# skyepurchase/MeatModeler

Measured on AMD Instinct MI355X. Metric: descriptor-match pairs/sec + BA residuals/sec, 500×1080p frames, 1/2/4/8 GPU, higher is better.
Workload: dtype u8/int32 (match), f64 (BA); 1 GPU; 500 frames 1920x1080, 4000 ORB kpts/frame, BF Hamming 2-NN + ratio, track linking, 2-view DLT, full BA (TRF, Schur, f64 MFMA Cholesky); frames=500, height=1080, width=1920, nfeatures=4000, parallelism=pairs/points x1

## Files before the change

meatmodeler_amd/csrc/schur.hip:

```cpp
#include "ba_eval.h"
#include "chol_init.h"

namespace {

constexpr int SR_WIN = 256;

__global__ __launch_bounds__(256) void point_inverse_kernel(int P, const double *__restrict__ Cd,
                                                            double *__restrict__ Cinv) {
    int p = blockIdx.x * 256 + threadIdx.x;
    if (p >= P) return;
    const double *c = Cd + (size_t)p * 6;
    const double a = c[0], b = c[1], d = c[2], e = c[3], f = c[4], g = c[5];
    const double m00 = e * g - f * f, m01 = d * f - b * g, m02 = b * f - d * e;
    const double det = a * m00 + b * m01 + d * m02;
    const double id = 1.0 / det;
    double *o = Cinv + (size_t)p * 6;
    o[0] = m00 * id;
    o[1] = m01 * id;
    o[2] = m02 * id;
    o[3] = (a * g - d * d) * id;
    o[4] = (b * d - a * f) * id;
    o[5] = (a * e - b * b) * id;
}

// ... 35 lines not shown
        }
        if (blockIdx.y == 0) {
            const double g0 = gp[(size_t)p * 3], g1 = gp[(size_t)p * 3 + 1], g2 = gp[(size_t)p * 3 + 2];
#pragma unroll
            for (int a = 0; a < 6; ++a) vg[a] += Y[a][0] * g0 + Y[a][1] * g1 + Y[a][2] * g2;
        }
        for (int e2i = pb.pt_ptr[p]; e2i < pb.pt_ptr[p + 1]; ++e2i) {
            const int o2 = pb.pt_obs[e2i];
            const int f2 = pb.fi[o2];
            if (f2 < w0 || f2 >= w0 + wn) continue;
            Proj p2;
            ba_eval<true, true>(cams + (size_t)f2 * 6, Xp, Ks, pb.obs[2 * (size_t)o2], pb.obs[2 * (size_t)o2 + 1], p2);
            double *dst = &acc[0][(f2 - w0) * 6];
#pragma unroll
            for (int b = 0; b < 6; ++b) {
                const double e0 = p2.Jc[0][b] * p2.Jp[0][0] + p2.Jc[1][b] * p2.Jp[1][0];
                const double e1 = p2.Jc[0][b] * p2.Jp[0][1] + p2.Jc[1][b] * p2.Jp[1][1];
                const double e2 = p2.Jc[0][b] * p2.Jp[0][2] + p2.Jc[1][b] * p2.Jp[1][2];
#pragma unroll
                for (int a = 0; a < 6; ++a)
                    atomicAdd(dst + a * (SR_WIN * 6) + b, Y[a][0] * e0 + Y[a][1] * e1 + Y[a][2] * e2);
            }
        }
    }
    __syncthreads();
    for (int e = threadIdx.x; e < 6 * wn * 6; e += 256) {
        const int a = e / (wn * 6), c = e % (wn * 6);
        const int col = w0 * 6 + c;
        double val = -acc[a][c];
        if (col / 6 == i) val += Bd[(size_t)i * 36 + a * 6 + (col % 6)];
        S[((size_t)i * 6 + a) * n + col] = val;
    }
    if (blockIdx.y == 0) {
#pragma unroll
        for (int a = 0; a < 6; ++a) {
            const double s = block_sum<256>(vg[a], sm);
            if (threadIdx.x == 0) v[(size_t)i * 6 + a] = gc[(size_t)i * 6 + a] - s;
        }
    }
}

#ifndef MM_SP_WAVES
#define MM_SP_WAVES 1
#endif
constexpr int SP_WAVES = MM_SP_WAVES;
constexpr int MAX_SLABS = 64;
struct SlabSync {
    int32_t *ready;
    int32_t *done;
    int32_t seg_count[MAX_SLABS];
    int cams_per_slab;
};
constexpr int CAMTAB = 11;
__device__ __forceinline__ void write_chunk_desc(const mm_ba_problem &pb, int32_t *__restrict__ desc, int64_t first, int64_t stride) {
    for (int64_t k = first; k < pb.n_chunks; k += stride) {
        const int sidx = pb.chunk_seg[k], seg = pb.seg_ids[sidx];
        const int ci = seg / (pb.cam_span + 1), cdd = seg % (pb.cam_span + 1);
        const int c_first = pb.seg_chunk_ptr[sidx];
        int32_t *o = desc + 8 * k;
        o[0] = ci;
        o[1] = ci - cdd;
        o[2] = pb.chunk_begin[k];
        o[3] = pb.chunk_end[k];
        o[4] = sidx;
        o[5] = c_first;
        o[6] = pb.seg_chunk_ptr[sidx + 1] - c_first;
        o[7] = 0;
    }
}
__global__ __launch_bounds__(64) void cam_table_kernel(int F, const double *__restrict__ cams, double *__restrict__ tab,
                                                       int32_t *__restrict__ seg_done, int64_t n_seg, const double *__restrict__ K_lean,
                                                       mm_ba_problem pb, int32_t *__restrict__ desc) {
    const int f = blockIdx.x * 64 + threadIdx.x;
    for (int64_t k = f; k < n_seg; k += (int64_t)gridDim.x * 64) seg_done[k] = 0;
    if (desc) write_chunk_desc(pb, desc, f, (int64_t)gridDim.x * 64);
    if (f >= F) return;
    const double *c = cams + (size_t)f * 6;
    if (K_lean) {
        cam_table2_row(c, K_lean, tab + (size_t)f * CAMTAB2);
        return;
    }
    const CamCoef k = cam_coef_of(c);
    double *t = tab + (size_t)f * CAMTAB;
    for (int q = 0; q < 6; ++q) t[q] = c[q];
    t[6] = k.c;
    t[7] = k.a;
    t[8] = k.b;
    t[9] = k.a1;
    t[10] = k.b1;
}

__device__ __forceinline__ CamVals cam_vals_from_table(const double *__restrict__ t) {
    CamVals v;
    v.rx = uniform_f64(t[0]);
    v.ry = uniform_f64(t[1]);
    v.rz = uniform_f64(t[2]);
    v.tx = uniform_f64(t[3]);
    v.ty = uniform_f64(t[4]);
    v.tz = uniform_f64(t[5]);
    v.k.c = uniform_f64(t[6]);
    v.k.a = uniform_f64(t[7]);
    v.k.b = uniform_f64(t[8]);
    v.k.a1 = uniform_f64(t[9]);
    v.k.b1 = uniform_f64(t[10]);
    return v;
}

constexpr int RED_LD = 65;
__device__ __forceinline__ void wave_lds_barrier() {
    __builtin_amdgcn_fence(__ATOMIC_RELEASE, "wavefront");
    __builtin_amdgcn_wave_barrier();
    __builtin_amdgcn_fence(__ATOMIC_ACQUIRE, "wavefront");
}
__device__ __forceinline__ void wave_reduce_42(const double (&acc)[42], double *slab , int lane, double &out0,
                                               double &out1) {
#pragma unroll
    for (int h = 0; h < 2; ++h) {
#pragma unroll
        for (int q = 0; q < 21; ++q) slab[q * RED_LD + lane] = acc[21 * h + q];
        wave_lds_barrier();
        double s = 0.0;
        if (lane < 21) {
            const double *row = slab + lane * RED_LD;
            double s0 = 0.0, s1 = 0.0, s2 = 0.0, s3 = 0.0;
#pragma unroll
            for (int j = 0; j < 64; j += 4) {
                s0 += row[j];
                s1 += row[j + 1];
// ... 118 lines not shown
        if (writer && lane < 21) {
            tot0 = 0.0;
            tot1 = 0.0;
            for (int cc = 0; cc < n_ch; ++cc) {
                tot0 += __hip_atomic_load(partial + (size_t)(c_first + cc) * 42 + lane, __ATOMIC_RELAXED, __HIP_MEMORY_SCOPE_AGENT);
                tot1 += __hip_atomic_load(partial + (size_t)(c_first + cc) * 42 + 21 + lane, __ATOMIC_RELAXED, __HIP_MEMORY_SCOPE_AGENT);
            }
        }
    }
    if (!writer) return;
    if (lane < 21) {
#pragma unroll
        for (int h = 0; h < 2; ++h) {
            const int q = 21 * h + lane;
            const double sum = h == 0 ? tot0 : tot1;
            if (q < 36) {
                double val = -sum;
                if (d == 0) val += Bd[(size_t)i * 36 + q];
                __hip_atomic_store(S + ((size_t)i * 6 + q / 6) * n + (size_t)f2 * 6 + q % 6, val, __ATOMIC_RELAXED, __HIP_MEMORY_SCOPE_AGENT);
                if (d != 0)
                    __hip_atomic_store(S + ((size_t)f2 * 6 + q % 6) * n + (size_t)i * 6 + q / 6, val, __ATOMIC_RELAXED, __HIP_MEMORY_SCOPE_AGENT);
            } else if (d == 0) {
                __hip_atomic_store(v + (size_t)i * 6 + (q - 36), gc[(size_t)i * 6 + (q - 36)] - sum, __ATOMIC_RELAXED, __HIP_MEMORY_SCOPE_AGENT);
            }
        }
    }
    if (slabs.ready) {
        asm volatile("s_waitcnt vmcnt(0)" ::: "memory");
        __builtin_amdgcn_wave_barrier();
        if (lane == 0) {
            const int sl = i / slabs.cams_per_slab;
            if (atomicAdd(slabs.done + sl, 1) == slabs.seg_count[sl] - 1)
                __hip_atomic_store(slabs.ready + sl, 1, __ATOMIC_RELEASE, __HIP_MEMORY_SCOPE_AGENT);
        }
    }
}


struct CamPQ {
    double P[9], q[3];
};
__device__ __forceinline__ double fast_rcp(double x) {
    double y = __builtin_amdgcn_rcp(x);
    double e = fma(-x, y, 1.0);
    y = fma(y, e, y);
    e = fma(-x, y, 1.0);
    return fma(y, e, y);
}

struct LeanJ {
    double Jc[2][6];
    double Jp[2][3];
};
__device__ __forceinline__ void lean_eval(const CamPQ &c, const double *__restrict__ Ks, const double *__restrict__ Jr,
                                          double X0, double X1, double X2, LeanJ &o) {
    const double u0 = fma(c.P[0], X0, fma(c.P[1], X1, fma(c.P[2], X2, c.q[0])));
    const double u1 = fma(c.P[3], X0, fma(c.P[4], X1, fma(c.P[5], X2, c.q[1])));
    const double u2 = fma(c.P[6], X0, fma(c.P[7], X1, fma(c.P[8], X2, c.q[2])));
    const double iz = fast_rcp(u2);
    const double p[2] = {u0 * iz, u1 * iz};
#pragma unroll
    for (int m = 0; m < 2; ++m) {
#pragma unroll
        for (int k = 0; k < 3; ++k) {
            o.Jp[m][k] = fma(-p[m], c.P[6 + k], c.P[3 * m + k]) * iz;
            o.Jc[m][3 + k] = fma(-p[m], Ks[6 + k], Ks[3 * m + k]) * iz;
        }
        const double g0 = X1 * o.Jp[m][2] - X2 * o.Jp[m][1];
        const double g1 = X2 * o.Jp[m][0] - X0 * o.Jp[m][2];
        const double g2 = X0 * o.Jp[m][1] - X1 * o.Jp[m][0];
#pragma unroll
        for (int k = 0; k < 3; ++k) o.Jc[m][k] = fma(g0, Jr[k], fma(g1, Jr[3 + k], g2 * Jr[6 + k]));
    }
}

constexpr int SLAB2 = 32;
struct ChunkDesc {
    int32_t i, f2, e_begin, e_end, sidx, c_first, n_ch, pad;
};
template <bool FORCE>
__device__ __forceinline__ CamPQ cam_pq_scalar(const double *__restrict__ t) {
    CamPQ v;
#pragma unroll
    for (int k = 0; k < 9; ++k) v.P[k] = FORCE ? uniform_f64(t[k]) : t[k];
#pragma unroll
    for (int k = 0; k < 3; ++k) v.q[k] = FORCE ? uniform_f64(t[9 + k]) : t[9 + k];
    return v;
}
template <bool FORCE_UNIFORM>
__device__ __forceinline__ void schur_pairs_body(const mm_ba_problem pb, const double *__restrict__ camtab,
                                                                    const ChunkDesc *__restrict__ desc,
                                                                    const double *__restrict__ pts,
                                                                    const double *__restrict__ Cinv,
                                                                    const double *__restrict__ gp,
                                                                    double *partial, const double *__restrict__ Bd,
                                                                    const double *__restrict__ gc, double *S, double *v,
                                                                    int32_t *seg_done, SlabSync slabs, unsigned wg_begin,
                                                                    unsigned wg_total, const unsigned bx) {
    __shared__ double Ks[9];
    __shared__ double red[SP_WAVES][21 * RED_LD];
    __shared__ double jrs[SP_WAVES][SLAB2];
    if (threadIdx.x < 9) Ks[threadIdx.x] = pb.K[threadIdx.x];
    const int lane = threadIdx.x & 63;
    const int wv = __builtin_amdgcn_readfirstlane((int)(threadIdx.x >> 6));
    const unsigned gpos = bx + wg_begin;
    const unsigned wg = (gpos & 1) ? wg_total - 1 - (gpos >> 1) : (gpos >> 1);
    const int64_t c = (int64_t)wg * SP_WAVES + wv;
    const bool live = c < pb.n_chunks;
    ChunkDesc cd = {};
    if (live) cd = desc[c];
    if (FORCE_UNIFORM) {
        cd.i = __builtin_amdgcn_readfirstlane(cd.i);
        cd.f2 = __builtin_amdgcn_readfirstlane(cd.f2);
        cd.e_begin = __builtin_amdgcn_readfirstlane(cd.e_begin);
        cd.e_end = __builtin_amdgcn_readfirstlane(cd.e_end);
        cd.sidx = __builtin_amdgcn_readfirstlane(cd.sidx);
        cd.c_first = __builtin_amdgcn_readfirstlane(cd.c_first);
        cd.n_ch = __builtin_amdgcn_readfirstlane(cd.n_ch);
    }
    const int i = cd.i, f2 = cd.f2, d = cd.i - cd.f2, sidx = cd.sidx;
    const int e_begin = cd.e_begin, e_end = cd.e_end;
    auto point_of = [&](int e) { return pb.pair_p ? pb.pair_p[e] : pb.pi[pb.pair_o[e]]; };
    auto self_of = [&](int e) { return d == 0 && pb.pair_o[e] == pb.pair_o2[e]; };
    int e = e_begin + lane;
    int p_next = -1;
    bool self_next = false;
    if (live) {
        if (e < e_end) {
            p_next = point_of(e);
            self_next = self_of(e);
        }
        if (lane < 9) jrs[wv][lane] = camtab[(size_t)i * CAMTAB2 + 12 + lane];
        else if (lane >= 16 && lane < 25) jrs[wv][lane] = camtab[(size_t)f2 * CAMTAB2 + 12 + lane - 16];
    }
    __syncthreads();
    if (!live) return;
    const CamPQ cp_i = cam_pq_scalar<FORCE_UNIFORM>(camtab + (size_t)i * CAMTAB2), cp_2 = cam_pq_scalar<FORCE_UNIFORM>(camtab + (size_t)f2 * CAMTAB2);
    const double *Jr_i = jrs[wv], *Jr_2 = jrs[wv] + 16;
    double acc[42];
#pragma unroll
    for (int q = 0; q < 42; ++q) acc[q] = 0.0;
    auto load_xc = [&](int p, double (&x)[12]) {
        if (p >= 0) {
            const double *Xp = pts + (size_t)p * 3, *ci = Cinv + (size_t)p * 6;
            x[0] = Xp[0];
            x[1] = Xp[1];
            x[2] = Xp[2];
#pragma unroll
            for (int q = 0; q < 6; ++q) x[3 + q] = ci[q];
            if (d == 0) {
                x[9] = gp[(size_t)p * 3];
                x[10] = gp[(size_t)p * 3 + 1];
                x[11] = gp[(size_t)p * 3 + 2];
            }
        }
    };
    auto pair_body = [&](int p, bool self, const double (&x)[12]) {
        const double X0 = x[0], X1 = x[1], X2 = x[2];
        const double q00 = x[3], q01 = x[4], q02 = x[5], q11 = x[6], q12 = x[7], q22 = x[8];
        LeanJ a;
        lean_eval(cp_i, Ks, Jr_i, X0, X1, X2, a);
        double Z[2][3];
#pragma unroll
        for (int m = 0; m < 2; ++m) {
            Z[m][0] = a.Jp[m][0] * q00 + a.Jp[m][1] * q01 + a.Jp[m][2] * q02;
            Z[m][1] = a.Jp[m][0] * q01 + a.Jp[m][1] * q11 + a.Jp[m][2] * q12;
            Z[m][2] = a.Jp[m][0] * q02 + a.Jp[m][1] * q12 + a.Jp[m][2] * q22;
        }
        double M[2][2], T[2][6];
        if (d == 0) {
            if (self) {
                const double g0 = x[9], g1 = x[10], g2 = x[11];
                const double z0 = Z[0][0] * g0 + Z[0][1] * g1 + Z[0][2] * g2, z1 = Z[1][0] * g0 + Z[1][1] * g1 + Z[1][2] * g2;
#pragma unroll
                for (int q = 0; q < 6; ++q) acc[36 + q] += a.Jc[0][q] * z0 + a.Jc[1][q] * z1;
            }
#pragma unroll
            for (int m = 0; m < 2; ++m)
#pragma unroll
                for (int n_ = 0; n_ < 2; ++n_) M[m][n_] = Z[m][0] * a.Jp[n_][0] + Z[m][1] * a.Jp[n_][1] + Z[m][2] * a.Jp[n_][2];
#pragma unroll
            for (int b = 0; b < 6; ++b) {
                T[0][b] = M[0][0] * a.Jc[0][b] + M[0][1] * a.Jc[1][b];
                T[1][b] = M[1][0] * a.Jc[0][b] + M[1][1] * a.Jc[1][b];
            }
        } else {
            LeanJ b2;
            lean_eval(cp_2, Ks, Jr_2, X0, X1, X2, b2);
#pragma unroll
            for (int m = 0; m < 2; ++m)
#pragma unroll
                for (int n_ = 0; n_ < 2; ++n_) M[m][n_] = Z[m][0] * b2.Jp[n_][0] + Z[m][1] * b2.Jp[n_][1] + Z[m][2] * b2.Jp[n_][2];
#pragma unroll
            for (int b = 0; b < 6; ++b) {
                T[0][b] = M[0][0] * b2.Jc[0][b] + M[0][1] * b2.Jc[1][b];
                T[1][b] = M[1][0] * b2.Jc[0][b] + M[1][1] * b2.Jc[1][b];
            }
        }
#pragma unroll
        for (int q = 0; q < 6; ++q)
#pragma unroll
            for (int b = 0; b < 6; ++b) acc[q * 6 + b] += a.Jc[0][q] * T[0][b] + a.Jc[1][q] * T[1][b];
    };
    double xc[12];
    load_xc(p_next, xc);
    int p_cur = p_next;
    bool self_cur = self_next;
    {
        const int en = e + 64;
        p_next = en < e_end ? point_of(en) : -1;
        self_next = en < e_end && self_of(en);
    }
#pragma clang loop unroll(disable)
    for (; e - lane < e_end; e += 64) {
        double xn[12];
        load_xc(p_next, xn);
        const int p_nn_e = e + 128;
        const int p_nn = p_nn_e < e_end ? point_of(p_nn_e) : -1;
        const bool self_nn = p_nn_e < e_end && self_of(p_nn_e);
        if (p_cur >= 0) pair_body(p_cur, self_cur, xc);
#pragma unroll
        for (int q = 0; q < 12; ++q) xc[q] = xn[q];
        p_cur = p_next;
        self_cur = self_next;
        p_next = p_nn;
        self_next = self_nn;
    }
    double tot0, tot1;
    wave_reduce_42(acc, red[wv], lane, tot0, tot1);
    const int c_first = cd.c_first, n_ch = cd.n_ch;
    const size_t n = (size_t)pb.F * 6;
    bool writer = true;
    if (n_ch > 1) {
        if (lane < 21) {
            __hip_atomic_store(partial + (size_t)c * 42 + lane, tot0, __ATOMIC_RELAXED, __HIP_MEMORY_SCOPE_AGENT);
            __hip_atomic_store(partial + (size_t)c * 42 + 21 + lane, tot1, __ATOMIC_RELAXED, __HIP_MEMORY_SCOPE_AGENT);
        }
        asm volatile("s_waitcnt vmcnt(0)" ::: "memory");
        __builtin_amdgcn_wave_barrier();
        int last = 0;
        if (lane == 0) last = atomicAdd(seg_done + sidx, 1) == n_ch - 1;
        writer = __shfl(last, 0, 64) != 0;
        if (writer && lane < 21) {
            tot0 = 0.0;
            tot1 = 0.0;
            for (int cc = 0; cc < n_ch; ++cc) {
                tot0 += __hip_atomic_load(partial + (size_t)(c_first + cc) * 42 + lane, __ATOMIC_RELAXED, __HIP_MEMORY_SCOPE_AGENT);
                tot1 += __hip_atomic_load(partial + (size_t)(c_first + cc) * 42 + 21 + lane, __ATOMIC_RELAXED, __HIP_MEMORY_SCOPE_AGENT);
            }
        }
    }
    if (!writer) return;
    const bool through = slabs.ready != nullptr;
    if (lane < 21) {
#pragma unroll
        for (int h = 0; h < 2; ++h) {
            const int q = 21 * h + lane;
            const double sum = h == 0 ? tot0 : tot1;
            if (q < 36) {
                double val = -sum;
                if (d == 0) val += Bd[(size_t)i * 36 + q];
                double *dst = S + ((size_t)i * 6 + q / 6) * n + (size_t)f2 * 6 + q % 6;
                double *mir = S + ((size_t)f2 * 6 + q % 6) * n + (size_t)i * 6 + q / 6;
                if (through) {
                    __hip_atomic_store(dst, val, __ATOMIC_RELAXED, __HIP_MEMORY_SCOPE_AGENT);
                    if (d != 0) __hip_atomic_store(mir, val, __ATOMIC_RELAXED, __HIP_MEMORY_SCOPE_AGENT);
                } else {
                    *dst = val;
                    if (d != 0) *mir = val;
                }
            } else if (d == 0) {
                double *dst = v + (size_t)i * 6 + (q - 36);
                const double val = gc[(size_t)i * 6 + (q - 36)] - sum;
                if (through) __hip_atomic_store(dst, val, __ATOMIC_RELAXED, __HIP_MEMORY_SCOPE_AGENT);
                else *dst = val;
            }
        }
    }
    if (slabs.ready) {
        asm volatile("s_waitcnt vmcnt(0)" ::: "memory");
        __builtin_amdgcn_wave_barrier();
        if (lane == 0) {
            const int sl = i / slabs.cams_per_slab;
            if (atomicAdd(slabs.done + sl, 1) == slabs.seg_count[sl] - 1)
// ... 6 lines not shown
                                                                    const ChunkDesc *__restrict__ desc,
                                                                    const double *__restrict__ pts,
                                                                    const double *__restrict__ Cinv,
                                                                    const double *__restrict__ gp,
                                                                    double *partial, const double *__restrict__ Bd,
                                                                    const double *__restrict__ gc, double *S, double *v,
                                                                    int32_t *seg_done, SlabSync slabs, unsigned wg_begin,
                                                                    unsigned wg_total) {
    schur_pairs_body<false>(pb, camtab, desc, pts, Cinv, gp, partial, Bd, gc, S, v, seg_done, slabs, wg_begin, wg_total, blockIdx.x);
}
__global__ __launch_bounds__(256) void zero_batch_kernel(const mm_batch_prob *__restrict__ tab, const int32_t *__restrict__ list) {
    const mm_batch_prob &bp = tab[list[blockIdx.y]];
    if (blockIdx.x >= bp.g_zero) return;
    double2 *S2 = reinterpret_cast<double2 *>(bp.S);
    const int64_t n2 = bp.nc * bp.nc / 2;
    for (int64_t i = (int64_t)blockIdx.x * 256 + threadIdx.x; i < n2; i += (int64_t)bp.g_zero * 256) S2[i] = make_double2(0.0, 0.0);
}
__global__ __launch_bounds__(64 * SP_WAVES, 2) void schur_pairs_batch_kernel(const mm_batch_prob *__restrict__ tab, const int32_t *__restrict__ list) {
    const mm_batch_prob &bp = tab[list[blockIdx.y]];
    if (blockIdx.x >= bp.g_pairs) return;
    SlabSync none = {};
    schur_pairs_body<true>(bp.pb, bp.schur_camtab, (const ChunkDesc *)bp.schur_desc, bp.x + bp.nc, bp.Cinv, bp.g + bp.nc, bp.schur_partial, bp.Bd,
                     bp.g, bp.S, bp.v, bp.schur_seg_done, none, 0u, bp.g_pairs, blockIdx.x);
}




__global__ void slab_flag_kernel(int32_t *flags, int s) {
    __hip_atomic_store(flags + s, 1, __ATOMIC_RELEASE, __HIP_MEMORY_SCOPE_AGENT);
}

__global__ void schur_diag_fill_kernel(mm_ba_problem pb, const double *__restrict__ Bd, const double *__restrict__ gc,
                                       double *__restrict__ S, double *__restrict__ v) {
    const int i = blockIdx.x;
    if (pb.cam_ptr[i + 1] != pb.cam_ptr[i]) return;
    const size_t n = (size_t)pb.F * 6;
    if (threadIdx.x < 36) S[((size_t)i * 6 + threadIdx.x / 6) * n + (size_t)i * 6 + threadIdx.x % 6] = Bd[(size_t)i * 36 + threadIdx.x];
    if (threadIdx.x < 6) v[(size_t)i * 6 + threadIdx.x] = gc[(size_t)i * 6 + threadIdx.x];
}

struct PrepExtra {
    mm_damp_spec dmp;
    int zero_bwb;
    int chol_init;
    mm_chol_init_args init;
};
__device__ __forceinline__ void schur_prepare_body(mm_ba_problem pb, const double *__restrict__ cams,
                                                            double *__restrict__ Bd, const double *__restrict__ Cd,
                                                            const double *__restrict__ gc, double *__restrict__ Cinv,
                                                            double *__restrict__ S, double *__restrict__ v,
                                                            double *__restrict__ tab, int32_t *__restrict__ seg_done, bool lean,
                                                            int32_t *__restrict__ desc , const unsigned bx, const unsigned gx,
                                                            const PrepExtra *ex = nullptr) {
    const int b = (int)bx, tid = threadIdx.x;
    for (int64_t k = (int64_t)b * 256 + tid; k < pb.n_seg; k += (int64_t)gx * 256) seg_done[k] = 0;
    if (desc) write_chunk_desc(pb, desc, (int64_t)b * 256 + tid, (int64_t)gx * 256);
    const bool fold = ex && ex->dmp.B;
    double reg = 0.0;
    if (fold) {
        if (ex->dmp.gh2) {
            const double r = trf_damping_value(ex->dmp.gh2[0], ex->dmp.d11[0], ex->dmp.Delta);
            reg = fmax(r, ex->dmp.min_damping);
            if (b == 0 && tid == 0) {
                ex->dmp.damp_out[0] = r;
                ex->dmp.damp_out[1] = reg;
            }
        } else {
            reg = ex->dmp.reg[0];
        }
    }
    if (ex && ex->chol_init) mm_chol_init_body(ex->init, bx, gx);
    const size_t n = (size_t)pb.F * 6;
    if (ex && ex->zero_bwb >= 0) {
        const int nblk = (int)((n + 63) / 64);
        for (size_t r = bx; r < n; r += gx) {
            const int bi = (int)(r >> 6);
            const int lo = bi - ex->zero_bwb < 0 ? 0 : bi - ex->zero_bwb, hi = bi + ex->zero_bwb >= nblk ? nblk - 1 : bi + ex->zero_bwb;
            const size_t c0 = (size_t)lo * 64, c1 = (size_t)(hi + 1) * 64 < n ? (size_t)(hi + 1) * 64 : n;
            const size_t d0 = r / 6 * 6;
            for (size_t c = c0 + 2 * (size_t)tid; c < c1; c += 512)
                if (c < d0 || c >= d0 + 6) *reinterpret_cast<double2 *>(S + r * n + c) = double2{0.0, 0.0};
        }
    }
    const int f = b * 256 + tid;
    if (f < pb.F) {
        const double *c = cams + (size_t)f * 6;
        if (lean) {
            cam_table2_row(c, pb.K, tab + (size_t)f * CAMTAB2);
        } else {
            const CamCoef k = cam_coef_of(c);
            double *t = tab + (size_t)f * CAMTAB;
            for (int q = 0; q < 6; ++q) t[q] = c[q];
            t[6] = k.c;
            t[7] = k.a;
            t[8] = k.b;
            t[9] = k.a1;
            t[10] = k.b1;
        }
    }
    if (b < pb.F) {
        const bool empty = pb.cam_ptr[b + 1] == pb.cam_ptr[b];
        if (tid < 36) {
            double bd;
            if (fold) {
                bd = ex->dmp.B[(size_t)b * 36 + tid];
                if (tid % 7 == 0) {
                    const double s = ex->dmp.si[(size_t)b * 6 + tid / 7];
                    bd = fma(s * s, reg, bd);
                }
                Bd[(size_t)b * 36 + tid] = bd;
            } else {
                bd = Bd[(size_t)b * 36 + tid];
            }
            if (empty)
                S[((size_t)b * 6 + tid / 6) * n + (size_t)b * 6 + tid % 6] = bd;
            else if (ex && ex->zero_bwb >= 0)
                S[((size_t)b * 6 + tid / 6) * n + (size_t)b * 6 + tid % 6] = 0.0;
        }
        if (empty && tid < 6) v[(size_t)b * 6 + tid] = gc[(size_t)b * 6 + tid];
    }
    const int p = b * 256 + tid;
    if (p < pb.P) {
        double a, bq, d, e, ff, g;
        if (fold) {
            const double *c = ex->dmp.C + (size_t)p * 6;
            const double *sp = ex->dmp.si + n + (size_t)p * 3;
            a = fma(sp[0] * sp[0], reg, c[0]);
            bq = c[1];
            d = c[2];
            e = fma(sp[1] * sp[1], reg, c[3]);
            ff = c[4];
            g = fma(sp[2] * sp[2], reg, c[5]);
        } else {
            const double *c = Cd + (size_t)p * 6;
            a = c[0], bq = c[1], d = c[2], e = c[3], ff = c[4], g = c[5];
        }
        const double m00 = e * g - ff * ff, m01 = d * ff - bq * g, m02 = bq * ff - d * e;
        const double det = a * m00 + bq * m01 + d * m02;
        const double id = 1.0 / det;
        double *o = Cinv + (size_t)p * 6;
        o[0] = m00 * id;
        o[1] = m01 * id;
        o[2] = m02 * id;
        o[3] = (a * g - d * d) * id;
        o[4] = (bq * d - a * ff) * id;
        o[5] = (a * e - bq * bq) * id;
    }
}
__global__ __launch_bounds__(256) void schur_prepare_kernel(mm_ba_problem pb, const double *__restrict__ cams,
                                                            double *__restrict__ Bd, const double *__restrict__ Cd,
                                                            const double *__restrict__ gc, double *__restrict__ Cinv,
                                                            double *__restrict__ S, double *__restrict__ v,
                                                            double *__restrict__ tab, int32_t *__restrict__ seg_done, bool lean,
                                                            int32_t *__restrict__ desc) {
    schur_prepare_body(pb, cams, Bd, Cd, gc, Cinv, S, v, tab, seg_done, lean, desc, blockIdx.x, gridDim.x);
}
__global__ __launch_bounds__(256) void schur_prepare_damped_kernel(mm_ba_problem pb, const double *__restrict__ cams,
                                                                   double *__restrict__ Bd, const double *__restrict__ gc,
                                                                   double *__restrict__ Cinv, double *__restrict__ S,
                                                                   double *__restrict__ v, double *__restrict__ tab,
                                                                   int32_t *__restrict__ seg_done, int32_t *__restrict__ desc,
                                                                   PrepExtra ex) {
    schur_prepare_body(pb, cams, Bd, nullptr, gc, Cinv, S, v, tab, seg_done, true, desc, blockIdx.x, gridDim.x, &ex);
}
__global__ __launch_bounds__(256) void schur_prepare_batch_kernel(const mm_batch_prob *__restrict__ tab, const int32_t *__restrict__ list) {
    const mm_batch_prob &bp = tab[list[blockIdx.y]];
    if (blockIdx.x >= bp.g_prep) return;
    schur_prepare_body(bp.pb, bp.x, bp.Bd, bp.Cd, bp.g, bp.Cinv, bp.S, bp.v, bp.schur_camtab, bp.schur_seg_done, true, bp.schur_desc,
                       blockIdx.x, bp.g_prep);
}


__global__ __launch_bounds__(256) void pairs_count_kernel(mm_ba_problem pb, int32_t *__restrict__ cnt,
                                                          int32_t *__restrict__ span_out) {
    const int64_t o = (int64_t)blockIdx.x * 256 + threadIdx.x;
    int dmax = 0;
    if (o < pb.O) {
        const int f = pb.fi[o], p = pb.pi[o];
        int c = 0;
        for (int e = pb.pt_ptr[p]; e < pb.pt_ptr[p + 1]; ++e) {
            const int d = f - pb.fi[pb.pt_obs[e]];
            c += d >= 0;
            dmax = max(dmax, d);
        }
        cnt[o] = c;
    }
    for (int off = 32; off > 0; off >>= 1) dmax = max(dmax, __shfl_down(dmax, off, 64));
    if ((threadIdx.x & 63) == 0 && dmax > __hip_atomic_load(span_out, __ATOMIC_RELAXED, __HIP_MEMORY_SCOPE_AGENT)) atomicMax(span_out, dmax);
}

__global__ __launch_bounds__(256) void pairs_emit_kernel(mm_ba_problem pb, const int64_t *__restrict__ offsets, int span,
                                                         int32_t *__restrict__ key, int32_t *__restrict__ po,
                                                         int32_t *__restrict__ po2) {
    const int64_t o = (int64_t)blockIdx.x * 256 + threadIdx.x;
    if (o >= pb.O) return;
    const int f = pb.fi[o], p = pb.pi[o];
    int64_t w = offsets[o];
    for (int e = pb.pt_ptr[p]; e < pb.pt_ptr[p + 1]; ++e) {
        const int o2 = pb.pt_obs[e];
        const int d = f - pb.fi[o2];
        if (d < 0) continue;
        key[w] = f * (span + 1) + d;
        po[w] = (int32_t)o;
        po2[w] = o2;
        ++w;
    }
}

}

extern "C" int mm_ba_pairs_count(mm_ctx *ctx, const mm_ba_problem *pb, int32_t *cnt, int32_t *span_out) {
    if (!ctx) return MM_ERR_ARG;
    if (!pb || !cnt || !span_out || (pb->O > 0 && (!pb->fi || !pb->pi || !pb->pt_ptr || !pb->pt_obs)))
        return mm_fail(ctx, MM_ERR_ARG, "mm_ba_pairs_count: bad argument");
    MM_HIP(ctx, hipMemsetAsync(span_out, 0, sizeof(int32_t), ctx->stream));
    if (pb->O == 0) return MM_OK;
    MM_LAUNCH(ctx, "pairs_count_kernel", pairs_count_kernel, dim3((unsigned)((pb->O + 255) / 256)), dim3(256), 0, *pb, cnt,
              span_out);
    return MM_OK;
}

extern "C" int mm_ba_pairs_emit(mm_ctx *ctx, const mm_ba_problem *pb, const int64_t *offsets, int span, int32_t *key,
                                int32_t *pair_o, int32_t *pair_o2) {
    if (!ctx) return MM_ERR_ARG;
    if (!pb || !offsets || !key || !pair_o || !pair_o2 || span < 0) return mm_fail(ctx, MM_ERR_ARG, "mm_ba_pairs_emit: bad argument");
    if (pb->O == 0) return MM_OK;
    if ((int64_t)pb->F * (span + 1) > 0x7fffffffLL) return mm_fail(ctx, MM_ERR_ARG, "mm_ba_pairs_emit: F * (span + 1) overflows the key");
    MM_LAUNCH(ctx, "pairs_emit_kernel", pairs_emit_kernel, dim3((unsigned)((pb->O + 255) / 256)), dim3(256), 0, *pb, offsets,
              span, key, pair_o, pair_o2);
    return MM_OK;
}

extern "C" size_t mm_ba_schur_workspace_bytes(const mm_ba_problem *pb) {
    if (!pb || pb->n_chunks <= 0) return 0;
    return mm_align_up((size_t)pb->n_chunks * 42 * sizeof(double), 256)  +
           mm_align_up((size_t)pb->n_seg * sizeof(int32_t), 256)  +
           mm_align_up(2 * MAX_SLABS * sizeof(int32_t), 256)  +
           mm_align_up((size_t)pb->F * CAMTAB2 * sizeof(double), 256)  +
           mm_align_up((size_t)pb->n_chunks * 32, 256) ;
}

namespace {
bool schur_pairs_lean() {
    static const bool lean = [] {
        const char *e = getenv("MM_SCHUR_PAIRS");
        return !(e && e[0] == 'r');
    }();
    return lean;
}
#define MM_LAUNCH_PAIRS(ctx, grid, pbv, camtab_, desc_, ...)                                                             \
    do {                                                                                                                 \
        if (schur_pairs_lean())                                                                                          \
            MM_LAUNCH(ctx, "schur_pairs_kernel", schur_pairs_kernel<2>, grid, dim3(64 * SP_WAVES), 0, pbv, camtab_,      \
                      (const ChunkDesc *)(desc_), __VA_ARGS__);                                                          \
        else                                                                                                             \
            MM_LAUNCH(ctx, "schur_pairs_ref_kernel", schur_pairs_ref_kernel, grid, dim3(64 * SP_WAVES), 0, pbv, camtab_, \
                      __VA_ARGS__);                                                                                      \
    } while (0)
struct SchurWs {
    double *partial, *camtab;
    int32_t *seg_done, *slab_ready, *slab_done, *desc;
};
SchurWs carve_schur_ws(const mm_ba_problem *pb, void *ws) {
    SchurWs w;
    char *p = (char *)ws;
    w.partial = (double *)p;
    p += mm_align_up((size_t)pb->n_chunks * 42 * sizeof(double), 256);
    w.seg_done = (int32_t *)p;
    p += mm_align_up((size_t)pb->n_seg * sizeof(int32_t), 256);
    w.slab_ready = (int32_t *)p;
    w.slab_done = w.slab_ready + MAX_SLABS;
    p += mm_align_up(2 * MAX_SLABS * sizeof(int32_t), 256);
    w.camtab = (double *)p;
    p += mm_align_up((size_t)pb->F * CAMTAB2 * sizeof(double), 256);
    w.desc = (int32_t *)p;
    return w;
}
}

extern "C" int mm_ba_schur(mm_ctx *ctx, const mm_ba_problem *pb, const double *cams, const double *pts,
                           const double *Bd, const double *Cd, const double *gc, const double *gp, double *S, double *v,
                           double *Cinv, void *ws, size_t ws_bytes) {
    if (!ctx) return MM_ERR_ARG;
    if (!pb || pb->F < 0 || pb->P < 0 || pb->O < 0 || !pb->K) return mm_fail(ctx, MM_ERR_ARG, "mm_ba_schur: bad problem");
    if (!cams || !pts || !Bd || !Cd || !gc || !gp || !S || !v || !Cinv || !pb->pt_ptr || !pb->cam_ptr ||
        (pb->O > 0 && (!pb->pt_obs || !pb->cam_obs || !pb->fi || !pb->pi || !pb->obs)))
        return mm_fail(ctx, MM_ERR_ARG, "mm_ba_schur: null pointer");
    if (pb->F == 0) return MM_OK;
    if (pb->n_seg > 0 && pb->n_chunks > 0 && pb->seg_ids && pb->seg_chunk_ptr && pb->chunk_seg && pb->chunk_begin &&
        pb->chunk_end && pb->pair_o && pb->pair_o2) {
        if (!ws || ws_bytes < mm_ba_schur_workspace_bytes(pb)) return mm_fail(ctx, MM_ERR_WORKSPACE, "mm_ba_schur: workspace too small");
        MM_HIP(ctx, hipMemsetAsync(S, 0, (size_t)pb->F * 6 * pb->F * 6 * sizeof(double), ctx->stream));
        const int64_t wgs = (pb->n_chunks + SP_WAVES - 1) / SP_WAVES;
        const SchurWs w = carve_schur_ws(pb, ws);
        SlabSync none = {};
        const int prep = (pb->P + 255) / 256 > pb->F ? (pb->P + 255) / 256 : pb->F;
        MM_LAUNCH(ctx, "schur_prepare_kernel", schur_prepare_kernel, dim3(prep), dim3(256), 0, *pb, cams, const_cast<double *>(Bd), Cd, gc,
                  Cinv, S, v, w.camtab, w.seg_done, schur_pairs_lean(), schur_pairs_lean() ? w.desc : (int32_t *)nullptr);
        MM_LAUNCH_PAIRS(ctx, dim3((unsigned)wgs), *pb, (const double *)w.camtab, w.desc, pts, (const double *)Cinv, gp, w.partial, Bd, gc, S, v,
                        w.seg_done, none, 0u, (unsigned)wgs);
        return MM_OK;
    }
    if (pb->P > 0)
        MM_LAUNCH(ctx, "point_inverse_kernel", point_inverse_kernel, dim3((pb->P + 255) / 256), dim3(256), 0, pb->P, Cd,
                  Cinv);
    const int nwin = (pb->F + SR_WIN - 1) / SR_WIN;
    MM_LAUNCH(ctx, "schur_rows_kernel", schur_rows_kernel, dim3(pb->F, nwin), dim3(256), 0, *pb, cams, pts, Bd, Cinv, gc,
              gp, S, v);
    return MM_OK;
}

extern "C" int mm_ba_schur_solve(mm_ctx *ctx, const mm_ba_problem *pb, const double *cams, const double *pts,
                                 const double *Bd, const double *Cd, const double *gc, const double *gp, double *S,
                                 double *v, double *Cinv, int half_bandwidth, int32_t *info, void *ws_schur,
                                 size_t ws_schur_bytes, void *ws_chol, size_t ws_chol_bytes, int n_slabs,
                                 int cams_per_slab, const int64_t *slab_seg_ptr, const int64_t *slab_chunk_ptr) {
    if (!ctx) return MM_ERR_ARG;
    if (!pb || !info) return mm_fail(ctx, MM_ERR_ARG, "mm_ba_schur_solve: bad argument");
    const int n = pb->F * 6;
    const bool pairs_ok = pb->n_seg > 0 && pb->n_chunks > 0 && pb->seg_ids && pb->seg_chunk_ptr && pb->chunk_seg &&
                          pb->chunk_begin && pb->chunk_end && pb->pair_o && pb->pair_o2;
    const bool overlap = pairs_ok && n_slabs >= 2 && n_slabs <= MAX_SLABS && cams_per_slab >= 16 && slab_seg_ptr &&
                         slab_chunk_ptr && mm_chol_fused_eligible(n, half_bandwidth) && pb->P > 0;
    if (!overlap) {
        int rc = mm_ba_schur(ctx, pb, cams, pts, Bd, Cd, gc, gp, S, v, Cinv, ws_schur, ws_schur_bytes);
        if (rc) return rc;
        return mm_chol_solve_sym(ctx, S, n, v, half_bandwidth, 1, info, ws_chol, ws_chol_bytes);
    }
    if (!cams || !pts || !Bd || !Cd || !gc || !gp || !S || !v || !Cinv) return mm_fail(ctx, MM_ERR_ARG, "mm_ba_schur_solve: null pointer");
    if (!ws_schur || ws_schur_bytes < mm_ba_schur_workspace_bytes(pb)) return mm_fail(ctx, MM_ERR_WORKSPACE, "mm_ba_schur_solve: workspace too small");
    if (slab_seg_ptr[0] != 0 || slab_seg_ptr[n_slabs] != pb->n_seg || slab_chunk_ptr[0] != 0 || slab_chunk_ptr[n_slabs] != pb->n_chunks ||
        (int64_t)n_slabs * cams_per_slab < pb->F)
        return mm_fail(ctx, MM_ERR_ARG, "mm_ba_schur_solve: slab tables do not cover the problem");
    if (!ctx->aux) {
        int lo = 0, hi = 0;
        (void)hipDeviceGetStreamPriorityRange(&lo, &hi);
        MM_HIP(ctx, hipStreamCreateWithPriority(&ctx->aux, hipStreamNonBlocking, hi));
        MM_HIP(ctx, hipEventCreateWithFlags(&ctx->ev_fork, hipEventDisableTiming));
        MM_HIP(ctx, hipEventCreateWithFlags(&ctx->ev_join, hipEventDisableTiming));
    }
    const SchurWs w = carve_schur_ws(pb, ws_schur);
    MM_LAUNCH(ctx, "point_inverse_kernel", point_inverse_kernel, dim3((pb->P + 255) / 256), dim3(256), 0, pb->P, Cd, Cinv);
    SlabSync slabs = {};
    slabs.ready = w.slab_ready;
    slabs.done = w.slab_done;
    slabs.cams_per_slab = cams_per_slab;
    for (int sl = 0; sl < n_slabs; ++sl) slabs.seg_count[sl] = (int32_t)(slab_seg_ptr[sl + 1] - slab_seg_ptr[sl]);
    MM_LAUNCH(ctx, "cam_table_kernel", cam_table_kernel, dim3((pb->F + 63) / 64), dim3(64), 0, pb->F, cams, w.camtab, w.seg_done,
              (int64_t)pb->n_seg, schur_pairs_lean() ? pb->K : (const double *)nullptr, *pb,
              schur_pairs_lean() ? w.desc : (int32_t *)nullptr);
    MM_HIP(ctx, hipMemsetAsync(S, 0, (size_t)n * n * sizeof(double), ctx->stream));
// ... 7 lines not shown
        MM_LAUNCH_PAIRS(ctx, dim3(wg_first), *pb, (const double *)w.camtab, w.desc, pts, (const double *)Cinv, gp, w.partial, Bd, gc, S, v,
                        w.seg_done, slabs, 0u, wg_total);
    MM_HIP(ctx, hipEventRecord(ctx->ev_fork, ctx->stream));
    MM_HIP(ctx, hipStreamWaitEvent(ctx->aux, ctx->ev_fork, 0));
    {
        mm_stream_swap sw(ctx, ctx->aux);
        int rc = mm_chol_solve_gated(ctx, S, n, v, 1, half_bandwidth, info, ws_chol, ws_chol_bytes, w.slab_ready, cams_per_slab, pb->F, 2);
        if (rc) {
            (void)hipEventRecord(ctx->ev_join, ctx->aux);
            (void)hipStreamWaitEvent(sw.saved, ctx->ev_join, 0);
            return rc;
        }
        MM_HIP(ctx, hipEventRecord(ctx->ev_join, ctx->aux));
    }
    MM_LAUNCH_PAIRS(ctx, dim3(wg_total - wg_first), *pb, (const double *)w.camtab, w.desc, pts, (const double *)Cinv, gp, w.partial, Bd, gc, S, v,
                    w.seg_done, slabs, wg_first, wg_total);
    MM_HIP(ctx, hipStreamWaitEvent(ctx->stream, ctx->ev_join, 0));
    return MM_OK;
}

int mm_ba_schur_solve_damped(mm_ctx *ctx, const mm_ba_problem *pb, const double *cams, const double *pts, const mm_damp_spec *dmp,
                             double *Bd, double *Cd, const double *gc, const double *gp, double *S, double *v, double *Cinv,
                             int half_bandwidth, int32_t *info, void *ws_schur, size_t ws_schur_bytes, void *ws_chol,
                             size_t ws_chol_bytes) {
    if (!ctx) return MM_ERR_ARG;
    if (!pb || !dmp || !info || !cams || !pts || !Bd || !gc || !gp || !S || !v || !Cinv || !dmp->B || !dmp->C || !dmp->si ||
        (!dmp->gh2 && !dmp->reg) || (dmp->gh2 && (!dmp->d11 || !dmp->damp_out)))
        return mm_fail(ctx, MM_ERR_ARG, "mm_ba_schur_solve_damped: bad argument");
    const int n = pb->F * 6;
    static const bool off = [] { const char *e = getenv("MM_SCHUR_FOLD"); return e && atoi(e) == 0; }();
    mm_chol_init_args ia = {};
    int sides = 0, bwb = 0;
    const bool pairs_ok = pb->n_seg > 0 && pb->n_chunks > 0 && pb->seg_ids && pb->seg_chunk_ptr && pb->chunk_seg && pb->chunk_begin &&
                          pb->chunk_end && pb->pair_o && pb->pair_o2 && pb->P > 0 && schur_pairs_lean();
    const bool fold = !off && pairs_ok && ws_schur && ws_schur_bytes >= mm_ba_schur_workspace_bytes(pb) &&
                      mm_chol_init_plan(ctx, n, half_bandwidth, info, ws_chol, ws_chol_bytes, &ia, &sides, &bwb);
    if (!fold) {
        if (!Cd) return mm_fail(ctx, MM_ERR_ARG, "mm_ba_schur_solve_damped: the separate calls need Cd");
        int rc = dmp->gh2 ? mm_ba_damp_damping(ctx, pb->F, pb->P, dmp->B, dmp->C, dmp->si, dmp->gh2, dmp->d11, dmp->Delta, dmp->min_damping,
                                                dmp->damp_out, Bd, Cd)
                          : mm_ba_damp(ctx, pb->F, pb->P, dmp->B, dmp->C, dmp->si, dmp->reg, Bd, Cd);
        if (rc) return rc;
        return mm_ba_schur_solve(ctx, pb, cams, pts, Bd, Cd, gc, gp, S, v, Cinv, half_bandwidth, info, ws_schur, ws_schur_bytes, ws_chol,
                                 ws_chol_bytes, 0, 0, nullptr, nullptr);
    }
    const SchurWs w = carve_schur_ws(pb, ws_schur);
    PrepExtra ex = {};
    ex.dmp = *dmp;
    ex.zero_bwb = bwb;
    ex.chol_init = 1;
    ex.init = ia;
    const int prep = (pb->P + 255) / 256 > pb->F ? (pb->P + 255) / 256 : pb->F;
    MM_LAUNCH(ctx, "schur_prepare_kernel", schur_prepare_damped_kernel, dim3(prep), dim3(256), 0, *pb, cams, Bd, gc, Cinv, S, v, w.camtab,
              w.seg_done, w.desc, ex);
    const int64_t wgs = (pb->n_chunks + SP_WAVES - 1) / SP_WAVES;
    SlabSync none = {};
    MM_LAUNCH_PAIRS(ctx, dim3((unsigned)wgs), *pb, (const double *)w.camtab, w.desc, pts, (const double *)Cinv, gp, w.partial,
                    (const double *)Bd, gc, S, v, w.seg_done, none, 0u, (unsigned)wgs);
    mm_chol_init_done(ctx, ws_chol, sides);
    const int rc = mm_chol_solve_sym(ctx, S, n, v, half_bandwidth, 1, info, ws_chol, ws_chol_bytes);
    mm_chol_init_done(ctx, nullptr, 0);
    return rc;
}

int mm_batch_schur_setup(mm_ctx *ctx, mm_batch_prob *bp, void *ws_schur, size_t ws_schur_bytes) {
    const mm_ba_problem *pb = &bp->pb;
    if (!(pb->n_seg > 0 && pb->n_chunks > 0 && pb->seg_ids && pb->seg_chunk_ptr && pb->chunk_seg && pb->chunk_begin && pb->chunk_end &&
          pb->pair_o && pb->pair_o2 && pb->pair_p) || pb->P <= 0)
        return mm_fail(ctx, MM_ERR_ARG, "mm_ba_trf_batched: a problem without a co-observation pair list");
    if (!ws_schur || ws_schur_bytes < mm_ba_schur_workspace_bytes(pb)) return mm_fail(ctx, MM_ERR_WORKSPACE, "mm_ba_trf_batched: Schur workspace");
    const SchurWs w = carve_schur_ws(pb, ws_schur);
    bp->schur_partial = w.partial;
    bp->schur_camtab = w.camtab;
    bp->schur_seg_done = w.seg_done;
    bp->schur_desc = w.desc;
    bp->g_prep = (uint32_t)((pb->P + 255) / 256 > pb->F ? (pb->P + 255) / 256 : pb->F);
    bp->g_pairs = (uint32_t)((pb->n_chunks + SP_WAVES - 1) / SP_WAVES);
    const int64_t n2 = bp->nc * bp->nc / 2;
    const int64_t gz = (n2 + 2047) / 2048;
    bp->g_zero = (uint32_t)(gz < 1 ? 1 : (gz > 1024 ? 1024 : gz));
    return MM_OK;
}
int mm_batch_schur(mm_ctx *ctx, const mm_batch_prob *tab, const int32_t *list, int n_list, unsigned max_g_zero, unsigned max_g_prep,
                   unsigned max_g_pairs) {
    if (n_list <= 0) return MM_OK;
    MM_LAUNCH(ctx, "schur_zero_kernel", zero_batch_kernel, dim3(max_g_zero, (unsigned)n_list), dim3(256), 0, tab, list);
    MM_LAUNCH(ctx, "schur_prepare_kernel", schur_prepare_batch_kernel, dim3(max_g_prep, (unsigned)n_list), dim3(256), 0, tab, list);
    MM_LAUNCH(ctx, "schur_pairs_kernel", schur_pairs_batch_kernel, dim3(max_g_pairs, (unsigned)n_list), dim3(64 * SP_WAVES), 0, tab, list);
    return MM_OK;
}
```

Measured before the change: 9171 billion descriptor pairs/s (match stage).

## Pack four small off-diagonal Schur chunks into one wavefront

Result: no change. 9176 billion descriptor pairs/s (match stage), median of 3 (+0.1%).

```diff
diff --git a/meatmodeler_amd/csrc/schur.hip b/meatmodeler_amd/csrc/schur.hip
--- a/meatmodeler_amd/csrc/schur.hip
+++ b/meatmodeler_amd/csrc/schur.hip
@@ -111,20 +111,36 @@
     int cams_per_slab;
 };
 constexpr int CAMTAB = 11;
-__device__ __forceinline__ void write_chunk_desc(const mm_ba_problem &pb, int32_t *__restrict__ desc, int64_t first, int64_t stride) {
-    for (int64_t k = first; k < pb.n_chunks; k += stride) {
-        const int sidx = pb.chunk_seg[k], seg = pb.seg_ids[sidx];
-        const int ci = seg / (pb.cam_span + 1), cdd = seg % (pb.cam_span + 1);
-        const int c_first = pb.seg_chunk_ptr[sidx];
-        int32_t *o = desc + 8 * k;
-        o[0] = ci;
-        o[1] = ci - cdd;
-        o[2] = pb.chunk_begin[k];
-        o[3] = pb.chunk_end[k];
-        o[4] = sidx;
-        o[5] = c_first;
-        o[6] = pb.seg_chunk_ptr[sidx + 1] - c_first;
-        o[7] = 0;
+constexpr int PACK_PAIRS = 16;
+__device__ __forceinline__ void write_chunk_desc(const mm_ba_problem &pb, int32_t *__restrict__ desc, int64_t first, int64_t stride,
+                                                 bool pack) {
+    const int lane = threadIdx.x & 63;
+    for (int64_t k = first; k - lane < pb.n_chunks; k += stride) {
+        const bool in = k < pb.n_chunks;
+        int ci = 0, cdd = 1, e_begin = 0, e_end = 0, sidx = 0, c_first = 0, n_ch = 1;
+        if (in) {
+            sidx = pb.chunk_seg[k];
+            const int seg = pb.seg_ids[sidx];
+            ci = seg / (pb.cam_span + 1), cdd = seg % (pb.cam_span + 1);
+            c_first = pb.seg_chunk_ptr[sidx];
+            n_ch = pb.seg_chunk_ptr[sidx + 1] - c_first;
+            e_begin = pb.chunk_begin[k];
+            e_end = pb.chunk_end[k];
+        }
+        int packed = pack && n_ch == 1 && cdd != 0 && e_end - e_begin <= PACK_PAIRS;
+        packed &= __shfl_xor(packed, 1, 64);
+        packed &= __shfl_xor(packed, 2, 64);
+        if (in) {
+            int32_t *o = desc + 8 * k;
+            o[0] = ci;
+            o[1] = ci - cdd;
+            o[2] = e_begin;
+            o[3] = e_end;
+            o[4] = sidx;
+            o[5] = c_first;
+            o[6] = n_ch;
+            o[7] = packed;
+        }
     }
 }
 __global__ __launch_bounds__(64) void cam_table_kernel(int F, const double *__restrict__ cams, double *__restrict__ tab,
@@ -132,7 +148,7 @@
                                                        mm_ba_problem pb, int32_t *__restrict__ desc) {
     const int f = blockIdx.x * 64 + threadIdx.x;
     for (int64_t k = f; k < n_seg; k += (int64_t)gridDim.x * 64) seg_done[k] = 0;
-    if (desc) write_chunk_desc(pb, desc, f, (int64_t)gridDim.x * 64);
+    if (desc) write_chunk_desc(pb, desc, f, (int64_t)gridDim.x * 64, false);
     if (f >= F) return;
     const double *c = cams + (size_t)f * 6;
     if (K_lean) {
@@ -357,7 +373,11 @@
     double Jc[2][6];
     double Jp[2][3];
 };
-__device__ __forceinline__ void lean_eval(const CamPQ &c, const double *__restrict__ Ks, const double *__restrict__ Jr,
+struct CamPQLds {
+    const double *P, *q;
+};
+template <class Cam>
+__device__ __forceinline__ void lean_eval(const Cam &c, const double *__restrict__ Ks, const double *__restrict__ Jr,
                                           double X0, double X1, double X2, LeanJ &o) {
     const double u0 = fma(c.P[0], X0, fma(c.P[1], X1, fma(c.P[2], X2, c.q[0])));
     const double u1 = fma(c.P[3], X0, fma(c.P[4], X1, fma(c.P[5], X2, c.q[1])));
@@ -381,8 +401,20 @@
 
 constexpr int SLAB2 = 32;
 struct ChunkDesc {
-    int32_t i, f2, e_begin, e_end, sidx, c_first, n_ch, pad;
+    int32_t i, f2, e_begin, e_end, sidx, c_first, n_ch, packed;
 };
+constexpr int QTAB = 2 * CAMTAB2;
+__device__ __forceinline__ double group_row_sum(const double *row) {
+    double s0 = 0.0, s1 = 0.0, s2 = 0.0, s3 = 0.0;
+#pragma unroll
+    for (int j = 0; j < 16; j += 4) {
+        s0 += row[j];
+        s1 += row[j + 1];
+        s2 += row[j + 2];
+        s3 += row[j + 3];
+    }
+    return (s0 + s1) + (s2 + s3);
+}
 template <bool FORCE>
 __device__ __forceinline__ CamPQ cam_pq_scalar(const double *__restrict__ t) {
     CamPQ v;
@@ -405,6 +437,7 @@
     __shared__ double Ks[9];
     __shared__ double red[SP_WAVES][21 * RED_LD];
     __shared__ double jrs[SP_WAVES][SLAB2];
+    __shared__ double qtab[SP_WAVES][4 * QTAB];
     if (threadIdx.x < 9) Ks[threadIdx.x] = pb.K[threadIdx.x];
     const int lane = threadIdx.x & 63;
     const int wv = __builtin_amdgcn_readfirstlane((int)(threadIdx.x >> 6));
@@ -412,8 +445,12 @@
     const unsigned wg = (gpos & 1) ? wg_total - 1 - (gpos >> 1) : (gpos >> 1);
     const int64_t c = (int64_t)wg * SP_WAVES + wv;
     const bool live = c < pb.n_chunks;
-    ChunkDesc cd = {};
-    if (live) cd = desc[c];
+    const int64_t cs = live ? c : 0;
+    ChunkDesc cd = desc[cs];
+    const bool quad_first = (c & 3) == 0;
+    const int grp = lane >> 4, gl = lane & 15;
+    const bool grp_live = live && quad_first && c + grp < pb.n_chunks;
+    const int4 gd = *reinterpret_cast<const int4 *>(desc + (grp_live ? c + grp : cs));
     if (FORCE_UNIFORM) {
         cd.i = __builtin_amdgcn_readfirstlane(cd.i);
         cd.f2 = __builtin_amdgcn_readfirstlane(cd.f2);
@@ -422,7 +459,9 @@
         cd.sidx = __builtin_amdgcn_readfirstlane(cd.sidx);
         cd.c_first = __builtin_amdgcn_readfirstlane(cd.c_first);
         cd.n_ch = __builtin_amdgcn_readfirstlane(cd.n_ch);
-    }
+        cd.packed = __builtin_amdgcn_readfirstlane(cd.packed);
+    }
+    const bool packed = live && cd.packed != 0;
     const int i = cd.i, f2 = cd.f2, d = cd.i - cd.f2, sidx = cd.sidx;
     const int e_begin = cd.e_begin, e_end = cd.e_end;
     auto point_of = [&](int e) { return pb.pair_p ? pb.pair_p[e] : pb.pi[pb.pair_o[e]]; };
@@ -430,7 +469,7 @@
     int e = e_begin + lane;
     int p_next = -1;
     bool self_next = false;
-    if (live) {
+    if (live && !packed) {
         if (e < e_end) {
             p_next = point_of(e);
             self_next = self_of(e);
@@ -440,12 +479,11 @@
     }
     __syncthreads();
     if (!live) return;
-    const CamPQ cp_i = cam_pq_scalar<FORCE_UNIFORM>(camtab + (size_t)i * CAMTAB2), cp_2 = cam_pq_scalar<FORCE_UNIFORM>(camtab + (size_t)f2 * CAMTAB2);
-    const double *Jr_i = jrs[wv], *Jr_2 = jrs[wv] + 16;
+    if (packed && !quad_first) return;
     double acc[42];
 #pragma unroll
     for (int q = 0; q < 42; ++q) acc[q] = 0.0;
-    auto load_xc = [&](int p, double (&x)[12]) {
+    auto load_xc = [&](int p, bool diag, double (&x)[12]) {
         if (p >= 0) {
             const double *Xp = pts + (size_t)p * 3, *ci = Cinv + (size_t)p * 6;
             x[0] = Xp[0];
@@ -453,18 +491,19 @@
             x[2] = Xp[2];
 #pragma unroll
             for (int q = 0; q < 6; ++q) x[3 + q] = ci[q];
-            if (d == 0) {
+            if (diag) {
                 x[9] = gp[(size_t)p * 3];
                 x[10] = gp[(size_t)p * 3 + 1];
                 x[11] = gp[(size_t)p * 3 + 2];
             }
         }
     };
-    auto pair_body = [&](int p, bool self, const double (&x)[12]) {
+    auto pair_body = [&](const auto &ci, const auto &c2, const double *Jri, const double *Jr2, bool diag, bool self,
+                         const double (&x)[12]) {
         const double X0 = x[0], X1 = x[1], X2 = x[2];
         const double q00 = x[3], q01 = x[4], q02 = x[5], q11 = x[6], q12 = x[7], q22 = x[8];
         LeanJ a;
-        lean_eval(cp_i, Ks, Jr_i, X0, X1, X2, a);
+        lean_eval(ci, Ks, Jri, X0, X1, X2, a);
         double Z[2][3];
 #pragma unroll
         for (int m = 0; m < 2; ++m) {
@@ -473,7 +512,7 @@
             Z[m][2] = a.Jp[m][0] * q02 + a.Jp[m][1] * q12 + a.Jp[m][2] * q22;
         }
         double M[2][2], T[2][6];
-        if (d == 0) {
+        if (diag) {
             if (self) {
                 const double g0 = x[9], g1 = x[10], g2 = x[11];
                 const double z0 = Z[0][0] * g0 + Z[0][1] * g1 + Z[0][2] * g2, z1 = Z[1][0] * g0 + Z[1][1] * g1 + Z[1][2] * g2;
@@ -491,7 +530,7 @@
             }
         } else {
             LeanJ b2;
-            lean_eval(cp_2, Ks, Jr_2, X0, X1, X2, b2);
+            lean_eval(c2, Ks, Jr2, X0, X1, X2, b2);
 #pragma unroll
             for (int m = 0; m < 2; ++m)
 #pragma unroll
@@ -507,8 +546,51 @@
 #pragma unroll
             for (int b = 0; b < 6; ++b) acc[q * 6 + b] += a.Jc[0][q] * T[0][b] + a.Jc[1][q] * T[1][b];
     };
+    const size_t n = (size_t)pb.F * 6;
+    if (packed) {
+        const bool has = grp_live && gd.z + gl < gd.w;
+        const int p = point_of(has ? gd.z + gl : gd.z);
+        double tr[QTAB / 16];
+#pragma unroll
+        for (int t = 0; t < QTAB / 16; ++t) {
+            const int k = gl + 16 * t;
+            tr[t] = camtab[k < CAMTAB2 ? (size_t)gd.x * CAMTAB2 + k : (size_t)gd.y * CAMTAB2 + (k - CAMTAB2)];
+        }
+        double xc[12];
+        load_xc(p, false, xc);
+        double *tg = qtab[wv] + grp * QTAB;
+#pragma unroll
+        for (int t = 0; t < QTAB / 16; ++t) tg[gl + 16 * t] = tr[t];
+        wave_lds_barrier();
+        const CamPQLds cq_i = {tg, tg + 9}, cq_2 = {tg + CAMTAB2, tg + CAMTAB2 + 9};
+        if (has) pair_body(cq_i, cq_2, tg + 12, tg + CAMTAB2 + 12, false, false, xc);
+        double *slab = red[wv];
+        double t0[2], t1 = 0.0;
+#pragma unroll
+        for (int h = 0; h < 2; ++h) {
+#pragma unroll
+            for (int q = 0; q < 21; ++q)
+                if (21 * h + q < 36) slab[q * RED_LD + lane] = acc[21 * h + q];
+            wave_lds_barrier();
+            t0[h] = gl < (h == 0 ? 16 : 15) ? group_row_sum(slab + gl * RED_LD + 16 * grp) : 0.0;
+            if (h == 0 && gl < 5) t1 = group_row_sum(slab + (16 + gl) * RED_LD + 16 * grp);
+            wave_lds_barrier();
+        }
+        if (!grp_live) return;
+        auto put = [&](int q, double sum) {
+            const double val = -sum;
+            S[((size_t)gd.x * 6 + q / 6) * n + (size_t)gd.y * 6 + q % 6] = val;
+            S[((size_t)gd.y * 6 + q % 6) * n + (size_t)gd.x * 6 + q / 6] = val;
+        };
+        put(gl, t0[0]);
+        if (gl < 5) put(16 + gl, t1);
+        if (gl < 15) put(21 + gl, t0[1]);
+        return;
+    }
+    const CamPQ cp_i = cam_pq_scalar<FORCE_UNIFORM>(camtab + (size_t)i * CAMTAB2), cp_2 = cam_pq_scalar<FORCE_UNIFORM>(camtab + (size_t)f2 * CAMTAB2);
+    const double *Jr_i = jrs[wv], *Jr_2 = jrs[wv] + 16;
     double xc[12];
-    load_xc(p_next, xc);
+    load_xc(p_next, d == 0, xc);
     int p_cur = p_next;
     bool self_cur = self_next;
     {
@@ -519,11 +601,11 @@
 #pragma clang loop unroll(disable)
     for (; e - lane < e_end; e += 64) {
         double xn[12];
-        load_xc(p_next, xn);
+        load_xc(p_next, d == 0, xn);
         const int p_nn_e = e + 128;
         const int p_nn = p_nn_e < e_end ? point_of(p_nn_e) : -1;
         const bool self_nn = p_nn_e < e_end && self_of(p_nn_e);
-        if (p_cur >= 0) pair_body(p_cur, self_cur, xc);
+        if (p_cur >= 0) pair_body(cp_i, cp_2, Jr_i, Jr_2, d == 0, self_cur, xc);
 #pragma unroll
         for (int q = 0; q < 12; ++q) xc[q] = xn[q];
         p_cur = p_next;
@@ -534,7 +616,6 @@
     double tot0, tot1;
     wave_reduce_42(acc, red[wv], lane, tot0, tot1);
     const int c_first = cd.c_first, n_ch = cd.n_ch;
-    const size_t n = (size_t)pb.F * 6;
     bool writer = true;
     if (n_ch > 1) {
         if (lane < 21) {
@@ -647,10 +728,10 @@
                                                             double *__restrict__ S, double *__restrict__ v,
                                                             double *__restrict__ tab, int32_t *__restrict__ seg_done, bool lean,
                                                             int32_t *__restrict__ desc , const unsigned bx, const unsigned gx,
-                                                            const PrepExtra *ex = nullptr) {
+                                                            bool pack, const PrepExtra *ex = nullptr) {
     const int b = (int)bx, tid = threadIdx.x;
     for (int64_t k = (int64_t)b * 256 + tid; k < pb.n_seg; k += (int64_t)gx * 256) seg_done[k] = 0;
-    if (desc) write_chunk_desc(pb, desc, (int64_t)b * 256 + tid, (int64_t)gx * 256);
+    if (desc) write_chunk_desc(pb, desc, (int64_t)b * 256 + tid, (int64_t)gx * 256, pack);
     const bool fold = ex && ex->dmp.B;
     double reg = 0.0;
     if (fold) {
@@ -748,22 +829,23 @@
                                                             const double *__restrict__ gc, double *__restrict__ Cinv,
                                                             double *__restrict__ S, double *__restrict__ v,
                                                             double *__restrict__ tab, int32_t *__restrict__ seg_done, bool lean,
-                                                            int32_t *__restrict__ desc) {
-    schur_prepare_body(pb, cams, Bd, Cd, gc, Cinv, S, v, tab, seg_done, lean, desc, blockIdx.x, gridDim.x);
+                                                            int32_t *__restrict__ desc, bool pack) {
+    schur_prepare_body(pb, cams, Bd, Cd, gc, Cinv, S, v, tab, seg_done, lean, desc, blockIdx.x, gridDim.x, pack);
 }
 __global__ __launch_bounds__(256) void schur_prepare_damped_kernel(mm_ba_problem pb, const double *__restrict__ cams,
                                                                    double *__restrict__ Bd, const double *__restrict__ gc,
                                                                    double *__restrict__ Cinv, double *__restrict__ S,
                                                                    double *__restrict__ v, double *__restrict__ tab,
                                                                    int32_t *__restrict__ seg_done, int32_t *__restrict__ desc,
-                                                                   PrepExtra ex) {
-    schur_prepare_body(pb, cams, Bd, nullptr, gc, Cinv, S, v, tab, seg_done, true, desc, blockIdx.x, gridDim.x, &ex);
-}
-__global__ __launch_bounds__(256) void schur_prepare_batch_kernel(const mm_batch_prob *__restrict__ tab, const int32_t *__restrict__ list) {
+                                                                   PrepExtra ex, bool pack) {
+    schur_prepare_body(pb, cams, Bd, nullptr, gc, Cinv, S, v, tab, seg_done, true, desc, blockIdx.x, gridDim.x, pack, &ex);
+}
+__global__ __launch_bounds__(256) void schur_prepare_batch_kernel(const mm_batch_prob *__restrict__ tab, const int32_t *__restrict__ list,
+                                                                  bool pack) {
     const mm_batch_prob &bp = tab[list[blockIdx.y]];
     if (blockIdx.x >= bp.g_prep) return;
     schur_prepare_body(bp.pb, bp.x, bp.Bd, bp.Cd, bp.g, bp.Cinv, bp.S, bp.v, bp.schur_camtab, bp.schur_seg_done, true, bp.schur_desc,
-                       blockIdx.x, bp.g_prep);
+                       blockIdx.x, bp.g_prep, pack);
 }
 
 
@@ -843,6 +925,10 @@
         return !(e && e[0] == 'r');
     }();
     return lean;
+}
+bool schur_pack_on() {
+    const char *e = getenv("MM_SCHUR_PACK");
+    return !(e && atoi(e) == 0);
 }
 #define MM_LAUNCH_PAIRS(ctx, grid, pbv, camtab_, desc_, ...)                                                             \
     do {                                                                                                                 \
@@ -892,7 +978,7 @@
         SlabSync none = {};
         const int prep = (pb->P + 255) / 256 > pb->F ? (pb->P + 255) / 256 : pb->F;
         MM_LAUNCH(ctx, "schur_prepare_kernel", schur_prepare_kernel, dim3(prep), dim3(256), 0, *pb, cams, const_cast<double *>(Bd), Cd, gc,
-                  Cinv, S, v, w.camtab, w.seg_done, schur_pairs_lean(), schur_pairs_lean() ? w.desc : (int32_t *)nullptr);
+                  Cinv, S, v, w.camtab, w.seg_done, schur_pairs_lean(), schur_pairs_lean() ? w.desc : (int32_t *)nullptr, schur_pack_on());
         MM_LAUNCH_PAIRS(ctx, dim3((unsigned)wgs), *pb, (const double *)w.camtab, w.desc, pts, (const double *)Cinv, gp, w.partial, Bd, gc, S, v,
                         w.seg_done, none, 0u, (unsigned)wgs);
         return MM_OK;
@@ -1006,7 +1092,7 @@
     ex.init = ia;
     const int prep = (pb->P + 255) / 256 > pb->F ? (pb->P + 255) / 256 : pb->F;
     MM_LAUNCH(ctx, "schur_prepare_kernel", schur_prepare_damped_kernel, dim3(prep), dim3(256), 0, *pb, cams, Bd, gc, Cinv, S, v, w.camtab,
-              w.seg_done, w.desc, ex);
+              w.seg_done, w.desc, ex, schur_pack_on());
     const int64_t wgs = (pb->n_chunks + SP_WAVES - 1) / SP_WAVES;
     SlabSync none = {};
     MM_LAUNCH_PAIRS(ctx, dim3((unsigned)wgs), *pb, (const double *)w.camtab, w.desc, pts, (const double *)Cinv, gp, w.partial,
@@ -1039,7 +1125,8 @@
                    unsigned max_g_pairs) {
     if (n_list <= 0) return MM_OK;
     MM_LAUNCH(ctx, "schur_zero_kernel", zero_batch_kernel, dim3(max_g_zero, (unsigned)n_list), dim3(256), 0, tab, list);
-    MM_LAUNCH(ctx, "schur_prepare_kernel", schur_prepare_batch_kernel, dim3(max_g_prep, (unsigned)n_list), dim3(256), 0, tab, list);
+    MM_LAUNCH(ctx, "schur_prepare_kernel", schur_prepare_batch_kernel, dim3(max_g_prep, (unsigned)n_list), dim3(256), 0, tab, list,
+              schur_pack_on());
     MM_LAUNCH(ctx, "schur_pairs_kernel", schur_pairs_batch_kernel, dim3(max_g_pairs, (unsigned)n_list), dim3(64 * SP_WAVES), 0, tab, list);
     return MM_OK;
 }
```
